# plainerman/DiffDock-Pocket

Hardware: AMD Instinct MI355X
Metric: ligand poses/sec (40 samples x 20 steps) on 3dpf (higher is better)
Workload: dtype f32 (fc and G products: fp16 hi/lo split of both operands on v_mfma_f32_16x16x32_f16 - the row-stationary conv kernel - and v_mfma_f32_32x32x16_f16, fp32 accumulate; G between its two kernels as fp16 hi + continuation byte = 19 significant bits; the exact fp32 MFMA form is timed in other_workloads)

## Files before the change

diffdock_pocket_amd/csrc/ddp_gemm.hip:

```cpp
#include <hip/hip_runtime.h>
#include <stdint.h>
#include <type_traits>
#include <stdlib.h>

#include "ddp_hip.h"
#include "ddp_internal.h"

typedef float f32x2 __attribute__((ext_vector_type(2)));
typedef float f32x4 __attribute__((ext_vector_type(4)));

#define DDP_GEMM_THREADS 256
#define DDP_GEMM_ROWS 128

struct GemmOffs {
  int off[DDP_MAX_GEMM_BATCH];
};

template <int KT, int CPL>
__global__ __launch_bounds__(DDP_GEMM_THREADS, 2) void ddp_stage_a_kernel(const float* __restrict__ x, int ldx, int nrows,
                                                                           const int32_t* __restrict__ rows,
                                                                           const int32_t* __restrict__ nrows_dev, int out_rows,
                                                                           const GemmOffs offs, const float* __restrict__ w,
                                                                           int k, int ncols, float* __restrict__ out, int ldo) {
  constexpr int KP = (KT > 0) ? KT / 2 : 32;
// ... 225 lines not shown

template <int KT>
__global__ __launch_bounds__(DDP_GEMM_THREADS, 2) void ddp_stage_a_x3_kernel(const float* __restrict__ x, int ldx, int nrows,
                                                                              const int32_t* __restrict__ rows,
                                                                              const int32_t* __restrict__ nrows_dev, int out_rows,
                                                                              int mrows, const GemmOffs offs,
                                                                              const __bf16* __restrict__ w3, int ncols,
                                                                              float* __restrict__ out, int ldo) {
  if (nrows_dev) nrows = min(nrows, *nrows_dev);
  if ((int)blockIdx.y * mrows >= nrows) return;
  constexpr int KP = (KT + 15) / 16 * 16, NS = KP / 16, CT = DDP_SA3_CT;
  constexpr int XS = KP + 8;
  constexpr int NV = (32 * KT / 4 + DDP_GEMM_THREADS - 1) / DDP_GEMM_THREADS;
  constexpr int TS = 36;
  constexpr int NM = NS * 6;
  __shared__ __attribute__((aligned(16))) __bf16 xt[2][3][32 * XS];
  __shared__ __attribute__((aligned(16))) float st[4][2][32 * TS];
  const int z = (int)blockIdx.z, tid = (int)threadIdx.x;
  const int wave = tid >> 6, lane = tid & 63, r = lane & 31, hh = lane >> 5;
  const int col0 = ((int)blockIdx.x * 4 + wave) * (32 * CT);
  bf16x8 wr[CT][3][NS];
#pragma unroll
  for (int t = 0; t < CT; ++t) {
    const int c = min(col0 + 32 * t + r, ncols - 1);
#pragma unroll
    for (int p = 0; p < 3; ++p)
#pragma unroll
      for (int s2 = 0; s2 < NS; ++s2)
        wr[t][p][s2] = *reinterpret_cast<const bf16x8*>(w3 + (((((size_t)z * 3 + p) * NS + s2) * 2 + hh) * ncols + c) * 8);
  }
  if constexpr (KP > KT) {
    for (int i = tid; i < 2 * 3 * 32 * (KP - KT); i += DDP_GEMM_THREADS) {
      const int kk = i % (KP - KT), rr = (i / (KP - KT)) % 32, bp = i / ((KP - KT) * 32);
      xt[bp / 3][bp % 3][rr * XS + KT + kk] = (__bf16)0.f;
    }
  }
  const float* __restrict__ xb = x + offs.off[z];
  for (int R0 = (int)blockIdx.y * mrows; R0 < nrows; R0 += (int)gridDim.y * mrows) {
  const int R1 = min(nrows, R0 + mrows);
  const bool al4 = ((ldx | offs.off[z]) & 3) == 0 && (reinterpret_cast<size_t>(x) & 15) == 0;
  f32x4 xv[NV];
  auto fetch = [&](int row0) {
#pragma unroll
    for (int v = 0; v < NV; ++v) {
      const int i = tid + v * DDP_GEMM_THREADS;
      const int rr = min(i / (KT / 4), 31), q = i % (KT / 4);
      const int ri = min(row0 + rr, nrows - 1);
      const float* __restrict__ p = xb + (size_t)(rows ? rows[ri] : ri) * ldx + 4 * q;
      if (al4)
        xv[v] = *reinterpret_cast<const f32x4*>(p);
      else
        xv[v] = f32x4{p[0], p[1], p[2], p[3]};
    }
  };
  auto park = [&](int buf) {
#pragma unroll
    for (int v = 0; v < NV; ++v) {
      const int i = tid + v * DDP_GEMM_THREADS;
      if (i < 32 * (KT / 4)) {
        const int rr = i / (KT / 4), q = i % (KT / 4);
        bf16x4 h, m, l;
#pragma unroll
        for (int e = 0; e < 4; ++e) {
          const float f = xv[v][e];
          h[e] = (__bf16)f;
          const float r1 = f - (float)h[e];
          m[e] = (__bf16)r1;
          l[e] = (__bf16)(r1 - (float)m[e]);
        }
        *reinterpret_cast<bf16x4*>(&xt[buf][0][rr * XS + 4 * q]) = h;
        *reinterpret_cast<bf16x4*>(&xt[buf][1][rr * XS + 4 * q]) = m;
        *reinterpret_cast<bf16x4*>(&xt[buf][2][rr * XS + 4 * q]) = l;
      }
    }
  };
  float* pend_ob = nullptr;
  int pend_c0 = 0, pend_rows = 0, pend_buf = 0, pbuf = 0;
  int pend_ri[4] = {0, 0, 0, 0};
  f32x4 dv = {0.f, 0.f, 0.f, 0.f};
  auto drain_read = [&](int p) {
    if (pend_ob) dv = *reinterpret_cast<const f32x4*>(&st[wave][pend_buf][(8 * p + (lane >> 3)) * TS + 4 * (lane & 7)]);
  };
  auto drain_store = [&](int p) {
    if (pend_ob) {
      const int rr = 8 * p + (lane >> 3), c = pend_c0 + 4 * (lane & 7);
      if (rr < pend_rows && c < ncols) *reinterpret_cast<f32x4*>(&pend_ob[(size_t)pend_ri[p] * ldo + c]) = dv;
    }
  };
  fetch(R0);
  park(0);
  __syncthreads();
  int buf = 0;
  for (int row0 = R0; row0 < R1; row0 += 32, buf ^= 1) {
    const bool more = row0 + 32 < R1;
    if (more) fetch(row0 + 32);
    bf16x8 a[3][NS];
#pragma unroll
    for (int p = 0; p < 3; ++p)
#pragma unroll
      for (int s2 = 0; s2 < NS; ++s2) a[p][s2] = *reinterpret_cast<const bf16x8*>(&xt[buf][p][r * XS + 16 * s2 + 8 * hh]);
    float* __restrict__ ob = out + (size_t)z * out_rows * ldo;
    int blk_ri[4];
#pragma unroll
    for (int p = 0; p < 4; ++p) {
      const int ri = min(row0 + 8 * p + (lane >> 3), R1 - 1);
      blk_ri[p] = rows ? rows[ri] : ri;
    }
#pragma unroll
    for (int t = 0; t < CT; ++t) {
      f32x16 acc;
#pragma unroll
      for (int i = 0; i < 16; ++i) acc[i] = 0.f;
#pragma unroll
      for (int m = 0; m < NM; ++m) {
        constexpr int PA[6] = {2, 0, 1, 1, 0, 0}, PB[6] = {0, 2, 1, 0, 1, 0};
        const int pr = m / NS, s2 = m % NS;
        acc = __builtin_amdgcn_mfma_f32_32x32x16_bf16(a[PA[pr]][s2], wr[t][PB[pr]][s2], acc, 0, 0, 0);
        static_assert(NM / 4 >= 3 && NM % 4 == 0, "quarter schedule");
        if (m % (NM / 4) == 0) drain_read(m / (NM / 4));
        if (m % (NM / 4) == 2) drain_store(m / (NM / 4));
      }
      float* tl = st[wave][pbuf];
#pragma unroll
      for (int i = 0; i < 16; ++i) tl[((i & 3) + 8 * (i >> 2) + 4 * hh) * TS + r] = acc[i];
      pend_ob = ob;
#pragma unroll
      for (int p = 0; p < 4; ++p) pend_ri[p] = blk_ri[p];
      pend_c0 = col0 + 32 * t;
      pend_rows = R1 - row0;
      pend_buf = pbuf;
      pbuf ^= 1;
    }
    if (more) park(buf ^ 1);
    __syncthreads();
  }
#pragma unroll
  for (int p = 0; p < 4; ++p) {
    drain_read(p);
    drain_store(p);
  }
  __syncthreads();
  }
}

typedef _Float16 h8 __attribute__((ext_vector_type(8)));
typedef _Float16 h4 __attribute__((ext_vector_type(4)));
#ifndef DDP_SAH_CT_GH
#define DDP_SAH_CT_GH 4
#endif
#ifndef DDP_SAH_CT
#define DDP_SAH_CT 4
#endif

template <int KT, bool GH = false, bool G3 = false>
__global__ __launch_bounds__(DDP_GEMM_THREADS, 2) void ddp_stage_a_h2_kernel(const float* __restrict__ x, int ldx, int nrows,
                                                                              const int32_t* __restrict__ rows,
                                                                              const int32_t* __restrict__ nrows_dev, int out_rows,
                                                                              int mrows, const GemmOffs offs,
                                                                              const _Float16* __restrict__ wh, int ncols,
                                                                              float* __restrict__ out, int ldo, int32_t* range_flag,
                                                                              const int32_t* __restrict__ gh_dest = nullptr) {
  if (nrows_dev) nrows = min(nrows, *nrows_dev);
  if ((int)blockIdx.y * mrows >= nrows) return;
  constexpr int KP = (KT + 15) / 16 * 16, NS = KP / 16, CT = GH ? DDP_SAH_CT_GH : DDP_SAH_CT;
  constexpr int XS = KP + 8;
  constexpr int NV = (32 * KT / 4 + DDP_GEMM_THREADS - 1) / DDP_GEMM_THREADS;
  constexpr int TS = 36;
  constexpr int RS3 = 392;
  __shared__ __attribute__((aligned(16))) _Float16 xt[2][2][32 * XS];
  __shared__ __attribute__((aligned(16))) float st[G3 ? 1 : 4][2][G3 ? 4 : 32 * TS];
  __shared__ __attribute__((aligned(16))) char g3t[G3 ? 4 : 1][G3 ? 32 * RS3 : 16];
  const int z = (int)blockIdx.z, tid = (int)threadIdx.x;
  const int wave = tid >> 6, lane = tid & 63, r = lane & 31, hh = lane >> 5;
  const int col0 = ((int)blockIdx.x * 4 + wave) * (32 * CT);
  h8 wr[CT][2][NS];
#pragma unroll
  for (int t = 0; t < CT; ++t) {
    const int c = min(col0 + 32 * t + r, ncols - 1);
#pragma unroll
    for (int p = 0; p < 2; ++p)
#pragma unroll
      for (int s2 = 0; s2 < NS; ++s2)
        wr[t][p][s2] = *reinterpret_cast<const h8*>(wh + (((((size_t)z * 2 + p) * NS + s2) * 2 + hh) * ncols + c) * 8);
  }
  if constexpr (KP > KT) {
    for (int i = tid; i < 2 * 2 * 32 * (KP - KT); i += DDP_GEMM_THREADS) {
      const int kk = i % (KP - KT), rr = (i / (KP - KT)) % 32, bp = i / ((KP - KT) * 32);
      xt[bp / 2][bp % 2][rr * XS + KT + kk] = (_Float16)0.f;
    }
  }
  const float* __restrict__ xb = x + offs.off[z];
  float* __restrict__ ob = out + (size_t)z * out_rows * ldo;
  int cq[CT];
#pragma unroll
  for (int t = 0; t < CT; ++t) cq[t] = max(0, min(4 * (lane & 7), ncols - 4 - (col0 + 32 * t)));
  int gh_o[CT][2];
  bool gh_sp[CT];
  float gh_max = 0.f;
#pragma unroll
  for (int t = 0; t < CT; ++t) {
    gh_o[t][0] = gh_o[t][1] = 0;
    gh_sp[t] = false;
    if constexpr (GH) {
      const int g = min(col0 + 32 * t + 8 * (lane & 3), ncols - 8) >> 3;
      const int32_t* __restrict__ d = gh_dest + ((size_t)z * (ncols >> 3) + g) * 2;
      gh_o[t][0] = d[0] & ~3;
      gh_o[t][1] = d[1];
      gh_sp[t] = (d[0] & 1) != 0;
    }
  }
  unsigned sp3 = 0u;
  int g3_rr[3] = {0, 0, 0}, g3_pc[3] = {0, 0, 0};
  if constexpr (G3) {
    const int g = min(col0 + 8 * (lane & 15), ncols - 8) >> 3;
    sp3 = (unsigned)__ballot((gh_dest[((size_t)z * (ncols >> 3) + g) * 2] & 1) != 0) & 0xffffu;
#pragma unroll
    for (int j = 0; j < 3; ++j) {
      g3_rr[j] = (64 * j + lane) / 24;
      g3_pc[j] = (64 * j + lane) % 24;
    }
  }
  for (int R0 = (int)blockIdx.y * mrows; R0 < nrows; R0 += (int)gridDim.y * mrows) {
  const int R1 = min(nrows, R0 + mrows);
  const bool al4 = ((ldx | offs.off[z]) & 3) == 0 && (reinterpret_cast<size_t>(x) & 15) == 0;
  f32x4 xv[NV];
  auto fetch = [&](int row0) {
#pragma unroll
    for (int v = 0; v < NV; ++v) {
      const int i = tid + v * DDP_GEMM_THREADS;
      const int rr = min(i / (KT / 4), 31), q = i % (KT / 4);
      const int ri = min(row0 + rr, nrows - 1);
      const float* __restrict__ p = xb + (size_t)(rows ? rows[ri] : ri) * ldx + 4 * q;
      if (al4)
        xv[v] = *reinterpret_cast<const f32x4*>(p);
      else
        xv[v] = f32x4{p[0], p[1], p[2], p[3]};
    }
  };
  auto park = [&](int buf) {
#pragma unroll
    for (int v = 0; v < NV; ++v) {
      const int i = tid + v * DDP_GEMM_THREADS;
      if (i < 32 * (KT / 4)) {
        const int rr = i / (KT / 4), q = i % (KT / 4);
        h4 h, l;
#pragma unroll
        for (int e = 0; e < 4; ++e) {
          const float f = GH ? xv[v][e] * (float)DDP_GH_SX : xv[v][e];
          if (!(fabsf(f) <= 65504.f) && range_flag) *range_flag = 1;
          h[e] = (_Float16)f;
          l[e] = (_Float16)(GH ? f - (float)h[e] : (f - (float)h[e]) * 2048.f);
        }
        *reinterpret_cast<h4*>(&xt[buf][0][rr * XS + 4 * q]) = h;
        *reinterpret_cast<h4*>(&xt[buf][1][rr * XS + 4 * q]) = l;
      }
    }
  };
  size_t pend_off[4] = {0, 0, 0, 0};
  int pend_lds[4] = {0, 0, 0, 0};
  bool pend_sp = false;
  int pbuf = 0;
  f32x4 dv = {0.f, 0.f, 0.f, 0.f};
  f32x4 dv2 = {0.f, 0.f, 0.f, 0.f};
  auto gh_read = [&](const float* pt, int p) {
    if (p & 1) {
      dv = dv2;
      return;
    }
    typedef float f32x8 __attribute__((ext_vector_type(8)));
    const f32x4 a = *reinterpret_cast<const f32x4*>(&pt[pend_lds[p]]), b = *reinterpret_cast<const f32x4*>(&pt[pend_lds[p] + 4]);
    const f32x8 f = {a[0], a[1], a[2], a[3], b[0], b[1], b[2], b[3]};
    const h8 hi = __builtin_convertvector(f, h8);
    const f32x8 rest = f - __builtin_convertvector(hi, f32x8);
    const h8 lo = __builtin_convertvector(rest, h8);
    const float m8 = fmaxf(fmaxf(fmaxf(fabsf(f[0]), fabsf(f[1])), fmaxf(fabsf(f[2]), fabsf(f[3]))), fmaxf(fmaxf(fabsf(f[4]), fabsf(f[5])), fmaxf(fabsf(f[6]), fabsf(f[7]))));
    gh_max = fmaxf(gh_max, pend_sp ? m8 : 0.f);
    const f32x4 vh = __builtin_bit_cast(f32x4, hi), vl = __builtin_bit_cast(f32x4, lo);
#pragma unroll
    for (int e = 0; e < 4; ++e) {
      dv[e] = pend_sp ? vh[e] : a[e];
      dv2[e] = pend_sp ? vl[e] : b[e];
    }
  };
  auto block = [&](auto drain_tag, int t, const h8 (&a)[2][NS], const int (&blk_ri)[4], int nr) {
    constexpr bool DRAIN = decltype(drain_tag)::value;
    f32x16 am, ac;
#pragma unroll
    for (int i = 0; i < 16; ++i) { am[i] = 0.f; ac[i] = 0.f; }
    const float* pt = st[wave][pbuf ^ 1];
#pragma unroll
    for (int s2 = 0; s2 < NS; ++s2) {
      if constexpr (DRAIN && NS == 4) {
        if constexpr (GH)
          gh_read(pt, s2);
        else
          dv = *reinterpret_cast<const f32x4*>(&pt[pend_lds[s2]]);
      }
      if constexpr (GH) {
        am = __builtin_amdgcn_mfma_f32_32x32x16_f16(wr[t][0][s2], a[0][s2], am, 0, 0, 0);
        am = __builtin_amdgcn_mfma_f32_32x32x16_f16(wr[t][1][s2], a[0][s2], am, 0, 0, 0);
        am = __builtin_amdgcn_mfma_f32_32x32x16_f16(wr[t][0][s2], a[1][s2], am, 0, 0, 0);
      } else {
        am = __builtin_amdgcn_mfma_f32_32x32x16_f16(a[0][s2], wr[t][0][s2], am, 0, 0, 0);
        ac = __builtin_amdgcn_mfma_f32_32x32x16_f16(a[0][s2], wr[t][1][s2], ac, 0, 0, 0);
        ac = __builtin_amdgcn_mfma_f32_32x32x16_f16(a[1][s2], wr[t][0][s2], ac, 0, 0, 0);
      }
      if constexpr (DRAIN && NS == 4) {
        {
          *reinterpret_cast<f32x4*>(&ob[pend_off[s2]]) = dv;
        }
      }
    }
    if constexpr (DRAIN && NS != 4) {
#pragma unroll
      for (int p = 0; p < 4; ++p) {
        if constexpr (GH)
          gh_read(pt, p);
        else
          dv = *reinterpret_cast<const f32x4*>(&pt[pend_lds[p]]);
        *reinterpret_cast<f32x4*>(&ob[pend_off[p]]) = dv;
      }
    }
    float* tl = st[wave][pbuf];
    if constexpr (GH) {
#pragma unroll
      for (int q4 = 0; q4 < 4; ++q4)
        *reinterpret_cast<f32x4*>(&tl[r * TS + 8 * q4 + 4 * hh]) = f32x4{am[4 * q4], am[4 * q4 + 1], am[4 * q4 + 2], am[4 * q4 + 3]};
    } else {
#pragma unroll
      for (int i = 0; i < 16; ++i) tl[((i & 3) + 8 * (i >> 2) + 4 * hh) * TS + r] = am[i] + ac[i] * (1.f / 2048.f);
    }
    if constexpr (GH) {
#if defined(DDP_GH_ABL) && DDP_GH_ABL == 1
      pend_sp = false;
#else
      pend_sp = gh_sp[t];
#endif
#pragma unroll
      for (int p = 0; p < 4; ++p) {
        const int rr = min(16 * (p >> 1) + (lane >> 2), nr - 1);
        pend_lds[p] = rr * TS + 8 * (lane & 3);
        pend_off[p] = (size_t)blk_ri[p >> 1] * ldo + gh_o[t][p & 1];
      }
    } else {
#pragma unroll
      for (int p = 0; p < 4; ++p) {
        const int rr = min(8 * p + (lane >> 3), nr - 1);
        pend_lds[p] = rr * TS + cq[t];
        pend_off[p] = (size_t)blk_ri[p] * ldo + (col0 + 32 * t + cq[t]);
      }
    }
    pbuf ^= 1;
  };
  auto block3 = [&](int t, const h8 (&a)[2][NS]) {
    f32x16 am;
#pragma unroll
    for (int i = 0; i < 16; ++i) am[i] = 0.f;
#pragma unroll
    for (int s2 = 0; s2 < NS; ++s2) {
      am = __builtin_amdgcn_mfma_f32_32x32x16_f16(wr[t][0][s2], a[0][s2], am, 0, 0, 0);
      am = __builtin_amdgcn_mfma_f32_32x32x16_f16(wr[t][1][s2], a[0][s2], am, 0, 0, 0);
      am = __builtin_amdgcn_mfma_f32_32x32x16_f16(wr[t][0][s2], a[1][s2], am, 0, 0, 0);
    }
    char* tl = g3t[G3 ? wave : 0] + r * RS3 + 96 * t;
#pragma unroll
    for (int q = 0; q < 4; ++q) {
      const bool sp = ((sp3 >> (4 * t + q)) & 1u) != 0u;
      const float v0 = am[4 * q], v1 = am[4 * q + 1], v2 = am[4 * q + 2], v3 = am[4 * q + 3];
      gh_max = fmaxf(gh_max, sp ? fmaxf(fmaxf(fabsf(v0), fabsf(v1)), fmaxf(fabsf(v2), fabsf(v3))) : 0.f);
      const uint32_t b0 = __builtin_bit_cast(uint32_t, v0) + 0x10u, b1 = __builtin_bit_cast(uint32_t, v1) + 0x10u;
      const uint32_t b2 = __builtin_bit_cast(uint32_t, v2) + 0x10u, b3 = __builtin_bit_cast(uint32_t, v3) + 0x10u;
      typedef __fp16 pk2 __attribute__((ext_vector_type(2)));
      const pk2 h01 = __builtin_amdgcn_cvt_pkrtz(__builtin_bit_cast(float, b0), __builtin_bit_cast(float, b1));
      const pk2 h23 = __builtin_amdgcn_cvt_pkrtz(__builtin_bit_cast(float, b2), __builtin_bit_cast(float, b3));
      const uint32_t lo = ((b0 >> 5) & 0xffu) | (((b1 >> 5) & 0xffu) << 8) | (((b2 >> 5) & 0xffu) << 16) | ((b3 >> 5) << 24);
      typedef uint32_t u32x2 __attribute__((ext_vector_type(2)));
      u32x2 w8;
      w8[0] = sp ? __builtin_bit_cast(uint32_t, h01) : __builtin_bit_cast(uint32_t, v0);
      w8[1] = sp ? __builtin_bit_cast(uint32_t, h23) : __builtin_bit_cast(uint32_t, v1);
      *reinterpret_cast<u32x2*>(tl + 24 * q + 8 * hh) = w8;
      *reinterpret_cast<uint32_t*>(tl + 24 * q + 16 + 4 * hh) = sp ? lo : __builtin_bit_cast(uint32_t, v2);
    }
  };
  auto drain3 = [&](int myrow, int nr) {
    __builtin_amdgcn_fence(__ATOMIC_RELEASE, "wavefront");
    __builtin_amdgcn_wave_barrier();
    const char* img = g3t[G3 ? wave : 0];
    float* __restrict__ oc = ob + 6 * (col0 >> 3);
#pragma unroll
    for (int p = 0; p < 4; ++p)
#pragma unroll
      for (int j = 0; j < 3; ++j) {
        const int rl = min(8 * p + g3_rr[j], nr - 1);
        typedef uint32_t u32x2 __attribute__((ext_vector_type(2)));
        const u32x2 lo8 = *reinterpret_cast<const u32x2*>(img + rl * RS3 + 16 * g3_pc[j]);
        const u32x2 hi8 = *reinterpret_cast<const u32x2*>(img + rl * RS3 + 16 * g3_pc[j] + 8);
        const int ri = __shfl(myrow, rl);
        typedef uint32_t u32x4 __attribute__((ext_vector_type(4)));
        *reinterpret_cast<u32x4*>(oc + (size_t)ri * ldo + 4 * g3_pc[j]) = u32x4{lo8[0], lo8[1], hi8[0], hi8[1]};
      }
    __builtin_amdgcn_wave_barrier();
  };
  fetch(R0);
  park(0);
  __syncthreads();
  int buf = 0;
  bool first = true;
  for (int row0 = R0; row0 < R1; row0 += 32, buf ^= 1) {
    const bool more = row0 + 32 < R1;
    if (more) fetch(row0 + 32);
    h8 a[2][NS];
#pragma unroll
    for (int p = 0; p < 2; ++p)
#pragma unroll
      for (int s2 = 0; s2 < NS; ++s2) a[p][s2] = *reinterpret_cast<const h8*>(&xt[buf][p][r * XS + 16 * s2 + 8 * hh]);
    int blk_ri[4];
#pragma unroll
    for (int p = 0; p < 4; ++p) {
      const int ri = min(row0 + (GH ? 16 * (p & 1) + (lane >> 2) : 8 * p + (lane >> 3)), R1 - 1);
      blk_ri[p] = rows ? rows[ri] : ri;
    }
    const int nr = R1 - row0;
    if constexpr (G3) {
      if (col0 < ncols) {
        const int ri = min(row0 + r, R1 - 1);
        const int myrow = rows ? rows[ri] : ri;
#pragma unroll
        for (int t = 0; t < CT; ++t) block3(t, a);
        drain3(myrow, nr);
      }
      if (more) park(buf ^ 1);
      __syncthreads();
      continue;
    }
#pragma unroll
    for (int t = 0; t < CT; ++t) {
      if (col0 + 32 * t >= ncols) continue;
      if (t == 0 && first)
        block(std::false_type{}, t, a, blk_ri, nr);
      else
        block(std::true_type{}, t, a, blk_ri, nr);
      first = false;
    }
    if (more) park(buf ^ 1);
    __syncthreads();
  }
  if (!first) {
    const float* pt = st[wave][pbuf ^ 1];
#pragma unroll
    for (int p = 0; p < 4; ++p) {
      if constexpr (GH)
        gh_read(pt, p);
      else
        dv = *reinterpret_cast<const f32x4*>(&pt[pend_lds[p]]);
      *reinterpret_cast<f32x4*>(&ob[pend_off[p]]) = dv;
    }
  }
  __syncthreads();
  }
  if constexpr (GH) {
    if (!(gh_max <= 65504.f) && range_flag) *range_flag = 1;
  }
}

static int stage_a_impl(const float* x, int ldx, int nrows, const int32_t* rows, const int32_t* nrows_dev, int out_rows,
                        const int32_t* offs, int nbatch, const float* w, const void* w_bf16x3, const void* w_h2, int k, int ncols, float* out,
                        int ldo, int32_t* range_flag, void* stream, const int32_t* gh_dest = nullptr, int gh_fmt = 0) {
  if (!rows) out_rows = nrows;
  if (out_rows < 1 && nrows > 0) return ddp_fail(DDP_EINVAL, "ddp_stage_a: out_rows");
  if (nbatch < 0 || nbatch > DDP_MAX_GEMM_BATCH) return ddp_fail(DDP_ELIMIT, "ddp_stage_a: nbatch > DDP_MAX_GEMM_BATCH");
  if (k < 2 || k > 64 || (k & 1)) return ddp_fail(DDP_ELIMIT, "ddp_stage_a: K must be even and in [2, 64]");
  if (ncols < 1 || nrows < 0 || (ldo < ncols && !(gh_dest && gh_fmt == 1 && ldo >= (ncols / 8) * 6)))
    return ddp_fail(DDP_EINVAL, "ddp_stage_a: ncols / nrows / ldo");
  if (gh_dest && gh_fmt == 1 && ((ncols & 127) != 0 || (ldo & 31) != 0))
    return ddp_fail(DDP_EINVAL, "ddp_stage_a_gh3: ncols % 128 == 0 (a wave's four column blocks), ldo % 32 == 0 (whole 128-byte lines)");
  if (nbatch == 0 || nrows == 0) return 0;
  if (!x || !offs || !w || !out) return ddp_fail(DDP_EINVAL, "ddp_stage_a: null argument");
  if ((reinterpret_cast<size_t>(x) & 3) || (reinterpret_cast<size_t>(out) & 7))
    return ddp_fail(DDP_EINVAL, "ddp_stage_a: x must be 4-byte aligned, out 8-byte aligned");
  GemmOffs O;
  for (int i = 0; i < DDP_MAX_GEMM_BATCH; ++i) O.off[i] = (i < nbatch) ? offs[i] : 0;
  hipStream_t s = (hipStream_t)stream;
  const int nry = (nrows + DDP_GEMM_ROWS - 1) / DDP_GEMM_ROWS;
#define DDP_GEMM_LAUNCH(KT, CPL)                                                                                 \
  hipLaunchKernelGGL((ddp_stage_a_kernel<KT, CPL>), dim3((ncols + CPL * DDP_GEMM_THREADS - 1) / (CPL * DDP_GEMM_THREADS), nry, nbatch), \
                     dim3(DDP_GEMM_THREADS), 0, s, x, ldx, nrows, rows, nrows_dev, out_rows, O, w, k, ncols, out, ldo)
  const bool wide = ((ncols | ldo) & 3) == 0 && ncols >= 4 * DDP_GEMM_THREADS && (reinterpret_cast<size_t>(out) & 15) == 0;
#define DDP_GEMM_MFMA(KT)                                                                                        \
  hipLaunchKernelGGL((ddp_stage_a_mfma_kernel<KT>), dim3((ncols + 128 * DDP_SA_CT - 1) / (128 * DDP_SA_CT), gy, nbatch), \
                     dim3(DDP_GEMM_THREADS), 0, s, x, ldx, nrows, rows, nrows_dev, out_rows, mrows, O, w, ncols, out, ldo)
  const bool listed = rows && nrows_dev;
  int mrows = listed ? (nrows >= 16384 ? 256 : 128) : (nrows >= 8192 ? DDP_GEMM_MROWS : nrows >= 384 ? 256 : 64);
  int gy = (nrows + mrows - 1) / mrows;
  if (listed && gy > 96) gy = 96;
#ifdef DDP_SA_TUNE
  if (nrows < 8192 || listed) {
    if (const char* e = getenv("DDP_SA_MROWS")) mrows = atoi(e);
    gy = (nrows + mrows - 1) / mrows;
    const char* c = getenv("DDP_SA_GYCAP");
    const int cap = c ? atoi(c) : 96;
    if (listed && gy > cap) gy = cap;
  }
#endif
  static const bool no_mfma = getenv("DDP_STAGE_A_VALU") != nullptr;
  if (gh_dest) {
    if (!(w_h2 && wide && (k == 60 || k == 32 || k == 24 || k == 16) && (reinterpret_cast<size_t>(w_h2) & 15) == 0 && (ncols & 31) == 0 &&
          (reinterpret_cast<size_t>(gh_dest) & 7) == 0))
      return ddp_fail(DDP_EINVAL, "ddp_stage_a_gh: plane output needs the h2 path (w_h2, k in {60, 32, 24, 16}) and ncols % 32 == 0");
    const dim3 grid((ncols + 128 * DDP_SAH_CT_GH - 1) / (128 * DDP_SAH_CT_GH), gy, nbatch);
    const int pad = ddp_shape_stage_a_pad;
    static int pad_have[8] = {0, 0, 0, 0, 0, 0, 0, 0};
#define DDP_GEMM_GH(KT, I)                                                                                       \
    {                                                                                                            \
      if (pad > 0) {                                                                                             \
        const hipError_t ep = (gh_fmt == 1) ? ddp_need_lds(reinterpret_cast<const void*>(ddp_stage_a_h2_kernel<KT, true, true>), pad, &pad_have[4 + I]) \
                                            : ddp_need_lds(reinterpret_cast<const void*>(ddp_stage_a_h2_kernel<KT, true>), pad, &pad_have[I]); \
        if (ep != hipSuccess) return ddp_fail_hip(ep, "hipFuncSetAttribute(stage A)");                           \
      }                                                                                                          \
      if (gh_fmt == 1)                                                                                           \
        hipLaunchKernelGGL((ddp_stage_a_h2_kernel<KT, true, true>), grid, dim3(DDP_GEMM_THREADS), pad, s, x, ldx, nrows, rows, nrows_dev, out_rows, mrows, O, \
                           reinterpret_cast<const _Float16*>(w_h2), ncols, out, ldo, range_flag, gh_dest);       \
      else                                                                                                       \
        hipLaunchKernelGGL((ddp_stage_a_h2_kernel<KT, true>), grid, dim3(DDP_GEMM_THREADS), pad, s, x, ldx, nrows, rows, nrows_dev, out_rows, mrows, O, \
                           reinterpret_cast<const _Float16*>(w_h2), ncols, out, ldo, range_flag, gh_dest);       \
    }
    switch (k) {
      case 60: DDP_GEMM_GH(60, 0); break;
      case 32: DDP_GEMM_GH(32, 1); break;
      case 24: DDP_GEMM_GH(24, 2); break;
      default: DDP_GEMM_GH(16, 3); break;
    }
#undef DDP_GEMM_GH
    const hipError_t eg = hipGetLastError();
    if (eg != hipSuccess) return ddp_fail_hip(eg, "ddp_stage_a_gh launch");
    return 0;
  }
  if (w_h2 && wide && (k == 60 || k == 32 || k == 24 || k == 16) && !no_mfma && (reinterpret_cast<size_t>(w_h2) & 15) == 0) {
    const dim3 grid((ncols + 128 * DDP_SAH_CT - 1) / (128 * DDP_SAH_CT), gy, nbatch);
#define DDP_GEMM_H2(KT)                                                                                          \
    hipLaunchKernelGGL((ddp_stage_a_h2_kernel<KT>), grid, dim3(DDP_GEMM_THREADS), 0, s, x, ldx, nrows, rows, nrows_dev, out_rows, mrows, O, \
                       reinterpret_cast<const _Float16*>(w_h2), ncols, out, ldo, range_flag)
    switch (k) {
      case 60: DDP_GEMM_H2(60); break;
      case 32: DDP_GEMM_H2(32); break;
      case 24: DDP_GEMM_H2(24); break;
      default: DDP_GEMM_H2(16); break;
    }
#undef DDP_GEMM_H2
    const hipError_t eh = hipGetLastError();
    if (eh != hipSuccess) return ddp_fail_hip(eh, "ddp_stage_a (h2) launch");
    return 0;
  }
  if (w_bf16x3 && wide && (k == 60 || k == 32) && !no_mfma && (reinterpret_cast<size_t>(w_bf16x3) & 15) == 0) {
    const dim3 grid((ncols + 128 * DDP_SA3_CT - 1) / (128 * DDP_SA3_CT), gy, nbatch);
    if (k == 60)
      hipLaunchKernelGGL((ddp_stage_a_x3_kernel<60>), grid, dim3(DDP_GEMM_THREADS), 0, s, x, ldx, nrows, rows, nrows_dev, out_rows, mrows, O,
                         reinterpret_cast<const __bf16*>(w_bf16x3), ncols, out, ldo);
    else
      hipLaunchKernelGGL((ddp_stage_a_x3_kernel<32>), grid, dim3(DDP_GEMM_THREADS), 0, s, x, ldx, nrows, rows, nrows_dev, out_rows, mrows, O,
                         reinterpret_cast<const __bf16*>(w_bf16x3), ncols, out, ldo);
    const hipError_t e3 = hipGetLastError();
    if (e3 != hipSuccess) return ddp_fail_hip(e3, "ddp_stage_a (bf16x3) launch");
    return 0;
  }
  if (ncols >= 512 && !no_mfma && (k == 60 || k == 64 || k == 32 || k == 24 || k == 16)) {
    switch (k) {
      case 60: DDP_GEMM_MFMA(60); break;
      case 64: DDP_GEMM_MFMA(64); break;
      case 32: DDP_GEMM_MFMA(32); break;
      case 24: DDP_GEMM_MFMA(24); break;
      default: DDP_GEMM_MFMA(16); break;
    }
  } else
  switch (k) {
    case 60: if (wide) DDP_GEMM_LAUNCH(60, 4); else DDP_GEMM_LAUNCH(60, 2); break;
    case 32: DDP_GEMM_LAUNCH(32, 2); break;
    case 24: DDP_GEMM_LAUNCH(24, 2); break;
    case 16: DDP_GEMM_LAUNCH(16, 2); break;
    default: DDP_GEMM_LAUNCH(0, 2); break;
  }
#undef DDP_GEMM_LAUNCH
#undef DDP_GEMM_MFMA
  const hipError_t err = hipGetLastError();
  if (err != hipSuccess) return ddp_fail_hip(err, "ddp_stage_a launch");
  return 0;
}

extern "C" int ddp_stage_a(const float* x, int ldx, int nrows, const int32_t* rows, const int32_t* nrows_dev, int out_rows,
                           const int32_t* offs, int nbatch, const float* w, const void* w_bf16x3, int k, int ncols, float* out, int ldo,
                           void* stream) {
  return stage_a_impl(x, ldx, nrows, rows, nrows_dev, out_rows, offs, nbatch, w, w_bf16x3, nullptr, k, ncols, out, ldo, nullptr, stream);
}

extern "C" int ddp_stage_a_h2(const float* x, int ldx, int nrows, const int32_t* rows, const int32_t* nrows_dev, int out_rows,
                              const int32_t* offs, int nbatch, const float* w, const void* w_h2, int k, int ncols, float* out, int ldo,
                              int32_t* range_flag, void* stream) {
  return stage_a_impl(x, ldx, nrows, rows, nrows_dev, out_rows, offs, nbatch, w, nullptr, w_h2, k, ncols, out, ldo, range_flag, stream);
}

extern "C" int ddp_stage_a_gh(const float* x, int ldx, int nrows, const int32_t* rows, const int32_t* nrows_dev, int out_rows,
                              const int32_t* offs, int nbatch, const float* w, const void* w_h2, int k, int ncols, float* out, int ldo,
                              int32_t* range_flag, const int32_t* dest, void* stream) {
  if (!dest) return ddp_fail(DDP_EINVAL, "ddp_stage_a_gh: dest");
  return stage_a_impl(x, ldx, nrows, rows, nrows_dev, out_rows, offs, nbatch, w, nullptr, w_h2, k, ncols, out, ldo, range_flag, stream, dest);
}

extern "C" int ddp_stage_a_gh3(const float* x, int ldx, int nrows, const int32_t* rows, const int32_t* nrows_dev, int out_rows,
                               const int32_t* offs, int nbatch, const float* w, const void* w_h2, int k, int ncols, float* out, int ldo,
                               int32_t* range_flag, const int32_t* dest, void* stream) {
  if (!dest) return ddp_fail(DDP_EINVAL, "ddp_stage_a_gh3: dest");
  return stage_a_impl(x, ldx, nrows, rows, nrows_dev, out_rows, offs, nbatch, w, nullptr, w_h2, k, ncols, out, ldo, range_flag, stream, dest, 1);
}
```

include/ddp_hip.h:

```cpp
#ifndef DDP_HIP_H
#define DDP_HIP_H

#include <stdint.h>

#ifdef __cplusplus
extern "C" {
#endif

#define DDP_ABI_VERSION 17
#define DDP_EINVAL (-1)
#define DDP_ELIMIT (-2)

#define DDP_MAX_TASKS 9
#define DDP_MAX_BLOCKS 4
#define DDP_MAX_SEGS 3
#define DDP_MAX_NS 64
#define DDP_EDGE_TILE 64

enum ddp_feat_kind {
  DDP_F_SCALAR_S0 = 0,
  DDP_F_DOT = 1,
  DDP_F_SCALAR_S1 = 2,
  DDP_F_VEC_S0 = 3,
  DDP_F_CROSS = 4
// ... 61 lines not shown
  float* msg;
  const float* g[2];
  const int32_t* pos;
  const int32_t* n_edges_dev;
  const void* w1h;
  const void* w2h;
  int32_t* h2_range_flag;
  const void* wsh;
  const float* bsp;
  const void* gh[2];
  int32_t gh_fmt;
  int32_t rows_form;
  int32_t rows_bias_k;
  int32_t rows_seg0, rows_seg1, rows_nts;
} ddp_conv_task_t;
#define DDP_ROWS_SX 16
#define DDP_ROWS_SW 256
#define DDP_ROWS_SH 16
#define DDP_ROWS_SG 32
#define DDP_ROWS_KPERM(ks, hh, i) (32 * ((ks) >> 1) + ((8 * ((ks) & 1) + (i)) & 3) + 8 * ((8 * ((ks) & 1) + (i)) >> 2) + 4 * (hh))
#define DDP_ROWS16_POS(j) (16 * (((j) & 7) >> 2) + 4 * ((j) >> 3) + ((j) & 3))
#define DDP_GH3_LD(hid, gcp) ((((((hid) + 7) / 8) * (gcp) + ((gcp) + 5) / 6 + 15) / 16) * 96)
#define DDP_GH_LD(hid, gcp) ((((((hid) + 7) / 8) * 8 + 1) * (gcp) + 31) / 32 * 32)
int ddp_conv_messages(const ddp_conv_shape_t* shape, const ddp_conv_task_t* tasks, int ntasks, void* stream);

int ddp_conv_rows(const ddp_conv_shape_t* shape, const ddp_conv_task_t* tasks, int ntasks, void* stream);

typedef struct {
  const float* msg;
  const int32_t* rowptr;
  const float* bn_scale;
  const float* bn_shift;
  int32_t n_edges;
  const int32_t* rowmap;
  const int32_t* n_edges_dev;
} ddp_reduce_src_t;
int ddp_segment_reduce(float* x, int ldx, int n_nodes, int d_out, const ddp_reduce_src_t* srcs, int nsrc,
                       int accumulate, int n_rep, int rep_stride, void* stream);

int ddp_edge_featurize(const float* pos_a, const int32_t* ia, const float* pos_b, const int32_t* ib, int n_edges,
                       const int32_t* n_edges_dev, const float* offset, int k_rbf, float coeff, const float* pre,
                       const int32_t* pre_idx, int ld_pre, const float* pre2, int n_pre2, int ld_pre2, const float* w1d,
                       const float* w2, const float* b2, int ns, float* out, float* sh, void* stream);

#define DDP_MAX_FEATURIZE_JOBS 8
typedef struct {
  const float* pos_a;
  const int32_t* ia;
  const float* pos_b;
  const int32_t* ib;
  int32_t n_edges;
  const int32_t* n_edges_dev;
  const float* offset;
  int32_t k_rbf;
  float coeff;
  const float* pre;
  const int32_t* pre_idx;
  int32_t ld_pre;
  const float* pre2;
  int32_t n_pre2, ld_pre2;
  const float* w1d;
  const float* w2;
  const float* b2;
  int32_t ns;
  float* out;
  float* sh;
} ddp_featurize_job_t;
int ddp_edge_featurize_jobs(const ddp_featurize_job_t* jobs, int njobs, void* stream);

int ddp_torsion_sh(const float* sh_edge, const float* bond_vec, const int32_t* bond_of_edge, int n_edges,
                   const int32_t* n_edges_dev, float* out, const float* x, int ldx, int ns, const int32_t* b0,
                   const int32_t* b1, int n_bonds, float* bond_attr, void* stream);

typedef struct {
  const float* t[4];
  int32_t t_stride[4];
  float sig_min[4], sig_max[4];
  float* sigma[4];
  int32_t n_graphs;
  float* cut;
  float cut_mul, cut_add;
  float* graph_emb;
  int32_t sd;
  float emb_scale;
  const float* freq;
  const float* lig_pos;
  const int32_t* graph_ptr;
  float* center;
  struct {
    const float* pos;
    const int32_t* b0;
    const int32_t* b1;
    int32_t n;
    float* mid;
    float* vec;
  } bonds[2];
  struct {
    const int32_t* src;
    int32_t* dst;
    int32_t n;
  } copy[2];
} ddp_prologue_args_t;
int ddp_step_prologue(const ddp_prologue_args_t* args, void* stream);

typedef struct {
  const float* gp;
  int32_t ld_gp, n_graphs, ns, sd;
  const float* graph_emb;
  const float* w1[2];
  const float* b1[2];
  const float* w2[2];
  const float* b2[2];
  const float* sigma[2];
  const float* so3_table;
  int32_t so3_n;
  float so3_lo, so3_span;
  float* out[2];
} ddp_trrot_args_t;
int ddp_trrot_head(const ddp_trrot_args_t* args, void* stream);

typedef struct {
  const float* h;
  int32_t ld_h, n_bonds, ns;
  const float* w1;
  const float* w2;
  const float* sigma;
  const int32_t* graph_of_bond;
  const float* torus_table;
  int32_t torus_n;
  float torus_lo, torus_span;
  float* out;
} ddp_tor_args_t;
int ddp_tor_head(const ddp_tor_args_t* args, void* stream);

#define DDP_MAX_GEMM_BATCH 16
#define DDP_G_LD(hid, gcols) ((((((hid) + 3) / 4) * 4 + 1) * (gcols) + 31) / 32 * 32)
int ddp_stage_a(const float* x, int ldx, int nrows, const int32_t* rows, const int32_t* nrows_dev, int out_rows, const int32_t* offs,
                int nbatch, const float* w, const void* w_bf16x3, int k, int ncols, float* out, int ldo, void* stream);

int ddp_stage_a_h2(const float* x, int ldx, int nrows, const int32_t* rows, const int32_t* nrows_dev, int out_rows, const int32_t* offs,
                   int nbatch, const float* w, const void* w_h2, int k, int ncols, float* out, int ldo, int32_t* range_flag, void* stream);
int ddp_stage_a_gh(const float* x, int ldx, int nrows, const int32_t* rows, const int32_t* nrows_dev, int out_rows, const int32_t* offs,
                   int nbatch, const float* w, const void* w_h2, int k, int ncols, float* out, int ldo, int32_t* range_flag,
                   const int32_t* dest, void* stream);

int ddp_stage_a_gh3(const float* x, int ldx, int nrows, const int32_t* rows, const int32_t* nrows_dev, int out_rows, const int32_t* offs,
                    int nbatch, const float* w, const void* w_h2, int k, int ncols, float* out, int ldo, int32_t* range_flag,
                    const int32_t* dest, void* stream);

#define DDP_GH_SX 2

int ddp_set_occupancy_shaping(int rows_min_lds_bytes, int stage_a_lds_pad_bytes);

int ddp_pose_update(const float* pos_in, int n_samples, int n_atoms, const float* tr, const float* rot, const float* tor,
                    int n_tor, const int32_t* bonds, const uint8_t* mask_rotate, float* pos_out, void* stream);

int ddp_sidechain_update(const float* pos_in, int n_samples, int n_atoms, const float* angles, int n_bonds,
                         const int32_t* edge_idx, const int32_t* subcomponents, const int32_t* mapping, float* pos_out,
                         void* stream);

typedef struct {
  const float* score[4];
  const float* z[4];
  float* out[4];
  int32_t n[4];
} ddp_sde_args_t;
int ddp_sde_update(const float* coef, const ddp_sde_args_t* args, void* stream);

#define DDP_RADIUS_DROP_SELF 1
#define DDP_RADIUS_NEAREST 2
int ddp_radius_count(const float* x, const int32_t* x_ptr, const float* y, const int32_t* y_batch, int ny, float r,
                     int max_neighbors, int flags, int32_t* counts, void* stream);
int ddp_radius_fill(const float* x, const int32_t* x_ptr, const float* y, const int32_t* y_batch, int ny, float r,
                    int max_neighbors, int flags, const int32_t* offsets, int32_t* out_query, int32_t* out_x, void* stream);
int ddp_knn(const float* x, const int32_t* x_ptr, const int32_t* batch, int n, int k, int32_t* out_neighbors, void* stream);

int ddp_group_by_key(const int32_t* key, int n_items, int n_keys, const int32_t* pay0, const int32_t* pay1, const int32_t* pay2,
                     int32_t* rowptr, int32_t* perm, int32_t* out_key, int32_t* out0, int32_t* out1, int32_t* out2,
                     int32_t* scratch, void* stream);

#define DDP_MAX_LIST_JOBS 12

typedef struct {
  int32_t n;
  const int32_t* n_dev;
  const int32_t* flag;
  const int32_t* val;
  const int32_t* rowptr;
  int32_t base;
  int32_t* excl;
  int32_t* excl2;
  int32_t* list;
  int32_t* total;
} ddp_scan_job_t;
int ddp_scan_jobs(const ddp_scan_job_t* jobs, int njobs, void* stream);

typedef struct {
  const int32_t* idx;
  int32_t n;
  const int32_t* n_dev;
  int32_t* mask;
} ddp_mark_job_t;
int ddp_mark_jobs(const ddp_mark_job_t* jobs, int njobs, void* stream);

typedef struct {
  int32_t n_rows;
  const int32_t* keep;
  const int32_t* old_rowptr;
  const int32_t* new_rowptr;
  const int32_t* in[3];
  int32_t* out[3];
} ddp_rowcopy_job_t;
int ddp_rowcopy_jobs(const ddp_rowcopy_job_t* jobs, int njobs, void* stream);

typedef struct {
  int32_t n;
  const int32_t* n_dev;
  const int32_t* mask_a;
  const int32_t* idx_a;
  const int32_t* mask_b;
  const int32_t* idx_b;
  int32_t* out_idx;
  const int32_t* pay[4];
  int32_t pay_add[4];
  int32_t* out[4];
  int32_t* total;
  int32_t* block_count;
  int32_t* block_off;
} ddp_select_job_t;
int ddp_select_jobs(const ddp_select_job_t* jobs, int njobs, void* stream);

int ddp_gather_rows(const float* x, int ldx, const int32_t* idx, int n, const int32_t* n_dev, float* out, int ldo, int ncols,
                    void* stream);

int ddp_clean_pair_maps(const int32_t* touched, const int32_t* recv, const int32_t* src, const int32_t* rowptr, int n_edges, int e0,
                        int n_graphs, int n0, int32_t* rowmap, int32_t* rows_v, void* stream);

int ddp_flex_mark(const float* pos, const int32_t* flag, int n_b_per_graph, const int32_t* a, const int32_t* b, int n_edges, int e0,
                  int n_a_per_graph, int a_too, int ref_list, int32_t* mark, void* stream);
int ddp_fallback_rowmap(const int32_t* mark, const int32_t* recv, const int32_t* old_rowptr, const int32_t* new_rowptr, int n_edges,
                        int n_recv_per_graph, int32_t* rowmap, void* stream);

typedef struct {
  const float* x;
  const int32_t* x_ptr;
  const float* y;
  const int32_t* y_batch;
  int32_t ny;
  float r;
  int32_t max_neighbors;
  int32_t flags;
  const float* graph_div;
  int32_t* counts;
  int32_t* offsets;
  int32_t base;
  int32_t* total;
  int32_t* out_query;
  int32_t* out_x;
  int32_t capacity;
  int32_t* overflow;
} ddp_radius_job_t;
int ddp_radius_search_jobs(const ddp_radius_job_t* jobs, int njobs, void* stream);

typedef struct {
  const int32_t* key;
  int32_t n_items;
  const int32_t* n_items_dev;
  int32_t n_keys;
  const int32_t* pay[3];
  int32_t* rowptr;
  int32_t* perm;
  int32_t* out_key;
  int32_t* out[3];
  const int32_t* key_map;
  int32_t* scratch;
} ddp_group_job_t;
int ddp_group_by_key_jobs(const ddp_group_job_t* jobs, int njobs, void* stream);

#define DDP_MAX_NODE_JOBS 8
#define DDP_MAX_NODE_CAT 16
typedef struct {
  int32_t n_rows;
  const int32_t* cat;
  int32_t ld_cat, n_cat;
  const float* table;
  int32_t feat_off[DDP_MAX_NODE_CAT];
  int32_t emb_dim, emb_mode;
  const float* dense[2];
  int32_t ld_dense[2], n_dense[2];
  const float* t;
  int32_t t_stride;
  float scale;
  const float* freq;
  const float* sig_emb;
  int32_t ld_sig, sd;
  float* sig_out;
  int32_t ld_sig_out;
  const float* w;
  const float* bias;
  float* out;
  int32_t ld_out, ncols, zero_to;
  const float* add;
  int32_t ld_add;
} ddp_node_job_t;
int ddp_node_linear(const ddp_node_job_t* jobs, int njobs, void* stream);

// ... 229 lines not shown
```

Measured before the change: 175.0.

## Add warp-specialized stage A G3 kernel with dedicated store-drain wave

Adds a new stage-A GEMM kernel for the G3 plane-output format. Three waves run the fp16 hi/lo MFMA blocks over 384-column tiles with double-buffered x staging, and a fourth wave only drains the LDS images to global memory, so stores overlap with compute. The host also caps the grid's y dimension to a persistent-style count based on CU slots, and the MFMA block is factored into a shared helper. The new path is gated to large row counts and can be toggled with an env var. The trade-off is one wave no longer doing MFMA, plus extra barriers per tile.

After: 178.7 (median of 6 runs). 2.1% higher.

```diff
diff --git a/diffdock_pocket_amd/csrc/ddp_gemm.hip b/diffdock_pocket_amd/csrc/ddp_gemm.hip
--- a/diffdock_pocket_amd/csrc/ddp_gemm.hip
+++ b/diffdock_pocket_amd/csrc/ddp_gemm.hip
@@ -401,6 +401,37 @@
 #define DDP_SAH_CT 4
 #endif
 
+template <int NS>
+__device__ __forceinline__ void sa_g3_block(const h8 (&w)[2][NS], const h8 (&a)[2][NS], char* tl, unsigned sp4, int hh, float& gh_max) {
+  f32x16 am;
+#pragma unroll
+  for (int i = 0; i < 16; ++i) am[i] = 0.f;
+#pragma unroll
+  for (int s2 = 0; s2 < NS; ++s2) {
+    am = __builtin_amdgcn_mfma_f32_32x32x16_f16(w[0][s2], a[0][s2], am, 0, 0, 0);
+    am = __builtin_amdgcn_mfma_f32_32x32x16_f16(w[1][s2], a[0][s2], am, 0, 0, 0);
+    am = __builtin_amdgcn_mfma_f32_32x32x16_f16(w[0][s2], a[1][s2], am, 0, 0, 0);
+  }
+#pragma unroll
+  for (int q = 0; q < 4; ++q) {
+    const bool sp = ((sp4 >> q) & 1u) != 0u;
+    const float v0 = am[4 * q], v1 = am[4 * q + 1], v2 = am[4 * q + 2], v3 = am[4 * q + 3];
+    gh_max = fmaxf(gh_max, sp ? fmaxf(fmaxf(fabsf(v0), fabsf(v1)), fmaxf(fabsf(v2), fabsf(v3))) : 0.f);
+    const uint32_t b0 = __builtin_bit_cast(uint32_t, v0) + 0x10u, b1 = __builtin_bit_cast(uint32_t, v1) + 0x10u;
+    const uint32_t b2 = __builtin_bit_cast(uint32_t, v2) + 0x10u, b3 = __builtin_bit_cast(uint32_t, v3) + 0x10u;
+    typedef __fp16 pk2 __attribute__((ext_vector_type(2)));
+    const pk2 h01 = __builtin_amdgcn_cvt_pkrtz(__builtin_bit_cast(float, b0), __builtin_bit_cast(float, b1));
+    const pk2 h23 = __builtin_amdgcn_cvt_pkrtz(__builtin_bit_cast(float, b2), __builtin_bit_cast(float, b3));
+    const uint32_t lo = ((b0 >> 5) & 0xffu) | (((b1 >> 5) & 0xffu) << 8) | (((b2 >> 5) & 0xffu) << 16) | ((b3 >> 5) << 24);
+    typedef uint32_t u32x2 __attribute__((ext_vector_type(2)));
+    u32x2 w8;
+    w8[0] = sp ? __builtin_bit_cast(uint32_t, h01) : __builtin_bit_cast(uint32_t, v0);
+    w8[1] = sp ? __builtin_bit_cast(uint32_t, h23) : __builtin_bit_cast(uint32_t, v1);
+    *reinterpret_cast<u32x2*>(tl + 24 * q + 8 * hh) = w8;
+    *reinterpret_cast<uint32_t*>(tl + 24 * q + 16 + 4 * hh) = sp ? lo : __builtin_bit_cast(uint32_t, v2);
+  }
+}
+
 template <int KT, bool GH = false, bool G3 = false>
 __global__ __launch_bounds__(DDP_GEMM_THREADS, 2) void ddp_stage_a_h2_kernel(const float* __restrict__ x, int ldx, int nrows,
                                                                               const int32_t* __restrict__ rows,
@@ -602,34 +633,7 @@
     pbuf ^= 1;
   };
   auto block3 = [&](int t, const h8 (&a)[2][NS]) {
-    f32x16 am;
-#pragma unroll
-    for (int i = 0; i < 16; ++i) am[i] = 0.f;
-#pragma unroll
-    for (int s2 = 0; s2 < NS; ++s2) {
-      am = __builtin_amdgcn_mfma_f32_32x32x16_f16(wr[t][0][s2], a[0][s2], am, 0, 0, 0);
-      am = __builtin_amdgcn_mfma_f32_32x32x16_f16(wr[t][1][s2], a[0][s2], am, 0, 0, 0);
-      am = __builtin_amdgcn_mfma_f32_32x32x16_f16(wr[t][0][s2], a[1][s2], am, 0, 0, 0);
-    }
-    char* tl = g3t[G3 ? wave : 0] + r * RS3 + 96 * t;
-#pragma unroll
-    for (int q = 0; q < 4; ++q) {
-      const bool sp = ((sp3 >> (4 * t + q)) & 1u) != 0u;
-      const float v0 = am[4 * q], v1 = am[4 * q + 1], v2 = am[4 * q + 2], v3 = am[4 * q + 3];
-      gh_max = fmaxf(gh_max, sp ? fmaxf(fmaxf(fabsf(v0), fabsf(v1)), fmaxf(fabsf(v2), fabsf(v3))) : 0.f);
-      const uint32_t b0 = __builtin_bit_cast(uint32_t, v0) + 0x10u, b1 = __builtin_bit_cast(uint32_t, v1) + 0x10u;
-      const uint32_t b2 = __builtin_bit_cast(uint32_t, v2) + 0x10u, b3 = __builtin_bit_cast(uint32_t, v3) + 0x10u;
-      typedef __fp16 pk2 __attribute__((ext_vector_type(2)));
-      const pk2 h01 = __builtin_amdgcn_cvt_pkrtz(__builtin_bit_cast(float, b0), __builtin_bit_cast(float, b1));
-      const pk2 h23 = __builtin_amdgcn_cvt_pkrtz(__builtin_bit_cast(float, b2), __builtin_bit_cast(float, b3));
-      const uint32_t lo = ((b0 >> 5) & 0xffu) | (((b1 >> 5) & 0xffu) << 8) | (((b2 >> 5) & 0xffu) << 16) | ((b3 >> 5) << 24);
-      typedef uint32_t u32x2 __attribute__((ext_vector_type(2)));
-      u32x2 w8;
-      w8[0] = sp ? __builtin_bit_cast(uint32_t, h01) : __builtin_bit_cast(uint32_t, v0);
-      w8[1] = sp ? __builtin_bit_cast(uint32_t, h23) : __builtin_bit_cast(uint32_t, v1);
-      *reinterpret_cast<u32x2*>(tl + 24 * q + 8 * hh) = w8;
-      *reinterpret_cast<uint32_t*>(tl + 24 * q + 16 + 4 * hh) = sp ? lo : __builtin_bit_cast(uint32_t, v2);
-    }
+    sa_g3_block<NS>(wr[t], a, g3t[G3 ? wave : 0] + r * RS3 + 96 * t, (sp3 >> (4 * t)) & 0xfu, hh, gh_max);
   };
   auto drain3 = [&](int myrow, int nr) {
     __builtin_amdgcn_fence(__ATOMIC_RELEASE, "wavefront");
@@ -710,6 +714,219 @@
   if constexpr (GH) {
     if (!(gh_max <= 65504.f) && range_flag) *range_flag = 1;
   }
+}
+
+#define DDP_SA_BAR()                                   \
+  do {                                                 \
+    asm volatile("s_waitcnt lgkmcnt(0)" ::: "memory"); \
+    __builtin_amdgcn_s_barrier();                      \
+    asm volatile("" ::: "memory");                     \
+  } while (0)
+template <int KT>
+__global__ __launch_bounds__(DDP_GEMM_THREADS, 2) void ddp_stage_a_g3dw_kernel(const float* __restrict__ x, int ldx, int nrows,
+                                                                                const int32_t* __restrict__ rows,
+                                                                                const int32_t* __restrict__ nrows_dev, int out_rows,
+                                                                                int mrows, const GemmOffs offs,
+                                                                                const _Float16* __restrict__ wh, int ncols,
+                                                                                float* __restrict__ out, int ldo, int32_t* range_flag,
+                                                                                const int32_t* __restrict__ gh_dest) {
+  static_assert(DDP_GEMM_THREADS == 256, "3 MFMA waves + 1 store wave");
+  if (nrows_dev) nrows = min(nrows, *nrows_dev);
+  if ((int)blockIdx.y * mrows >= nrows) return;
+  constexpr int KP = (KT + 15) / 16 * 16, NS = KP / 16;
+  constexpr int XS = KP + 8, RS3 = 392;
+  constexpr int NP = 32 * (KT / 4);
+  constexpr int NMT = 192, NV = (NP + NMT - 1) / NMT;
+  __shared__ __attribute__((aligned(16))) _Float16 xt[2][2][32 * XS];
+  __shared__ __attribute__((aligned(16))) char img[3][32 * RS3];
+  __shared__ int32_t rowid[2][32];
+  const int z = (int)blockIdx.z, tid = (int)threadIdx.x;
+  const int wave = __builtin_amdgcn_readfirstlane(tid >> 6), lane = tid & 63, r = lane & 31, hh = lane >> 5;
+  const int colw = (int)blockIdx.x * 384;
+  const int ngr = min(3, (ncols - colw) >> 7);
+  if constexpr (KP > KT) {
+    for (int i = tid; i < 2 * 2 * 32 * (KP - KT); i += DDP_GEMM_THREADS) {
+      const int kk = i % (KP - KT), rr = (i / (KP - KT)) % 32, bp = i / ((KP - KT) * 32);
+      xt[bp / 2][bp % 2][rr * XS + KT + kk] = (_Float16)0.f;
+    }
+  }
+  struct Tile { int R0, R1, row0; };
+  const int ystep = (int)gridDim.y * mrows;
+  auto tile_next = [&](Tile t) {
+    t.row0 += 32;
+    if (t.row0 >= t.R1) {
+      t.R0 += ystep;
+      t.row0 = t.R0;
+      t.R1 = min(nrows, t.R0 + mrows);
+    }
+    return t;
+  };
+  const Tile tile0 = {(int)blockIdx.y * mrows, min(nrows, (int)blockIdx.y * mrows + mrows), (int)blockIdx.y * mrows};
+  if (wave == 3) {
+    float* __restrict__ ob = out + (size_t)z * out_rows * ldo + 6 * (colw >> 3);
+    int dl[12];
+    size_t doff[12];
+#pragma unroll
+    for (int k = 0; k < 12; ++k) { dl[k] = 0; doff[k] = 0; }
+    auto drain = [&](int g) {
+      const char* im = img[g];
+      float* __restrict__ og = ob + 96 * g;
+#pragma unroll
+      for (int k = 0; k < 12; ++k) {
+        typedef uint32_t u32x2 __attribute__((ext_vector_type(2)));
+        typedef uint32_t u32x4 __attribute__((ext_vector_type(4)));
+        const u32x2 lo8 = *reinterpret_cast<const u32x2*>(im + dl[k]);
+        const u32x2 hi8 = *reinterpret_cast<const u32x2*>(im + dl[k] + 8);
+        *reinterpret_cast<u32x4*>(og + doff[k]) = u32x4{lo8[0], lo8[1], hi8[0], hi8[1]};
+      }
+    };
+    Tile t = tile0;
+    DDP_SA_BAR();
+    for (int n = 0;; ++n) {
+      if (n > 0 && ngr > 2) drain(2);
+      DDP_SA_BAR();
+      {
+        const int nr = t.R1 - t.row0;
+#pragma unroll
+        for (int k = 0; k < 12; ++k) {
+          const int i = 64 * (k % 3) + lane, rl = min(8 * (k / 3) + i / 24, nr - 1);
+          dl[k] = rl * RS3 + 16 * (i % 24);
+          doff[k] = (size_t)rowid[n & 1][rl] * ldo + 4 * (i % 24);
+        }
+      }
+      DDP_SA_BAR();
+      drain(0);
+      DDP_SA_BAR();
+      if (ngr > 1) drain(1);
+      DDP_SA_BAR();
+      t = tile_next(t);
+      if (t.row0 >= nrows) break;
+    }
+    if (ngr > 2) drain(2);
+    return;
+  }
+  h8 wr[4][2][NS];
+#pragma unroll
+  for (int j = 0; j < 4; ++j) {
+    const int c = min(colw + 32 * (3 * j + wave) + r, ncols - 1);
+#pragma unroll
+    for (int p = 0; p < 2; ++p)
+#pragma unroll
+      for (int s2 = 0; s2 < NS; ++s2)
+        wr[j][p][s2] = *reinterpret_cast<const h8*>(wh + (((((size_t)z * 2 + p) * NS + s2) * 2 + hh) * ncols + c) * 8);
+  }
+  unsigned sp3;
+  {
+    const int l = lane & 15;
+    const int g = min(((colw + 32 * (3 * (l >> 2) + wave)) >> 3) + (l & 3), (ncols >> 3) - 1);
+    sp3 = (unsigned)__ballot((gh_dest[((size_t)z * (ncols >> 3) + g) * 2] & 1) != 0) & 0xffffu;
+  }
+  float gh_max = 0.f;
+  const float* __restrict__ xb = x + offs.off[z];
+  const bool al4 = ((ldx | offs.off[z]) & 3) == 0 && (reinterpret_cast<size_t>(x) & 15) == 0;
+  auto run = [&](auto listed_tag, auto al4_tag) {
+  constexpr bool LISTED = decltype(listed_tag)::value, AL4 = decltype(al4_tag)::value;
+  f32x4 xv[NV];
+  int xrow[NV], xnext[NV];
+  auto rows_of = [&](int row0, int (&dst)[NV]) {
+#pragma unroll
+    for (int v = 0; v < NV; ++v) {
+      const int i = min(tid + v * NMT, NP - 1);
+      const int ri = min(row0 + i / (KT / 4), nrows - 1);
+      if constexpr (LISTED)
+        dst[v] = rows[ri];
+      else
+        dst[v] = ri;
+    }
+  };
+  auto fetch = [&]() {
+#pragma unroll
+    for (int v = 0; v < NV; ++v) {
+      const int i = min(tid + v * NMT, NP - 1);
+      const float* __restrict__ p = xb + (size_t)xrow[v] * ldx + 4 * (i % (KT / 4));
+      if constexpr (AL4)
+        xv[v] = *reinterpret_cast<const f32x4*>(p);
+      else
+        xv[v] = f32x4{p[0], p[1], p[2], p[3]};
+    }
+  };
+  auto park = [&](int buf) {
+#pragma unroll
+    for (int v = 0; v < NV; ++v) {
+      const int i = tid + v * NMT;
+      if (i < NP) {
+        const int rr = i / (KT / 4), q = i % (KT / 4);
+        h4 h, l;
+#pragma unroll
+        for (int e = 0; e < 4; ++e) {
+          const float f = xv[v][e] * (float)DDP_GH_SX;
+          if (!(fabsf(f) <= 65504.f) && range_flag) *range_flag = 1;
+          h[e] = (_Float16)f;
+          l[e] = (_Float16)(f - (float)h[e]);
+        }
+        *reinterpret_cast<h4*>(&xt[buf][0][rr * XS + 4 * q]) = h;
+        *reinterpret_cast<h4*>(&xt[buf][1][rr * XS + 4 * q]) = l;
+        if (q == 0) rowid[buf][rr] = xrow[v];
+      }
+    }
+  };
+  {
+    Tile t1 = tile_next(tile0), t2 = tile_next(t1);
+    rows_of(tile0.row0, xrow);
+    fetch();
+    park(0);
+    rows_of(t1.row0, xnext);
+    DDP_SA_BAR();
+    for (int n = 0;; ++n) {
+      const int buf = n & 1;
+      const bool more = t1.row0 < nrows;
+      if (more) {
+#pragma unroll
+        for (int v = 0; v < NV; ++v) xrow[v] = xnext[v];
+        fetch();
+        rows_of(t2.row0, xnext);
+      }
+      h8 a[2][NS];
+#pragma unroll
+      for (int p = 0; p < 2; ++p)
+#pragma unroll
+        for (int s2 = 0; s2 < NS; ++s2) a[p][s2] = *reinterpret_cast<const h8*>(&xt[buf][p][r * XS + 16 * s2 + 8 * hh]);
+#pragma unroll
+      for (int j = 0; j < 4; ++j) {
+        const int b = 3 * j + wave;
+        if ((b >> 2) < ngr)
+          sa_g3_block<NS>(wr[j], a, img[b >> 2] + r * RS3 + 96 * (b & 3), (sp3 >> (4 * j)) & 0xfu, hh, gh_max);
+        if (j == 3 && more) park(buf ^ 1);
+        DDP_SA_BAR();
+      }
+      if (!more) break;
+      t1 = t2;
+      t2 = tile_next(t2);
+    }
+  }
+  };
+  if (rows) {
+    if (al4)
+      run(std::true_type{}, std::true_type{});
+    else
+      run(std::true_type{}, std::false_type{});
+  } else {
+    if (al4)
+      run(std::false_type{}, std::true_type{});
+    else
+      run(std::false_type{}, std::false_type{});
+  }
+  if (!(gh_max <= 65504.f) && range_flag) *range_flag = 1;
+}
+
+extern "C" int ddp_sa_drainwave;
+int ddp_sa_drainwave = -1;
+static int stage_a_drainwave() {
+  if (ddp_sa_drainwave < 0) {
+    const char* e = getenv("DDP_SA_DRAINWAVE");
+    ddp_sa_drainwave = (e && e[0] == '0') ? 0 : (e && e[0] == '2') ? 2 : 1;
+  }
+  return ddp_sa_drainwave;
 }
 
 static int stage_a_impl(const float* x, int ldx, int nrows, const int32_t* rows, const int32_t* nrows_dev, int out_rows,
@@ -753,14 +970,44 @@
 #endif
   static const bool no_mfma = getenv("DDP_STAGE_A_VALU") != nullptr;
   if (gh_dest) {
-    if (!(w_h2 && wide && (k == 60 || k == 32 || k == 24 || k == 16) && (reinterpret_cast<size_t>(w_h2) & 15) == 0 && (ncols & 31) == 0 &&
+    const bool wide_gh = gh_fmt == 1 ? (((ncols | ldo) & 3) == 0 && (reinterpret_cast<size_t>(out) & 15) == 0) : wide;
+    if (!(w_h2 && wide_gh && (k == 60 || k == 32 || k == 24 || k == 16) && (reinterpret_cast<size_t>(w_h2) & 15) == 0 && (ncols & 31) == 0 &&
           (reinterpret_cast<size_t>(gh_dest) & 7) == 0))
       return ddp_fail(DDP_EINVAL, "ddp_stage_a_gh: plane output needs the h2 path (w_h2, k in {60, 32, 24, 16}) and ncols % 32 == 0");
-    const dim3 grid((ncols + 128 * DDP_SAH_CT_GH - 1) / (128 * DDP_SAH_CT_GH), gy, nbatch);
+    const int dw_mode = gh_fmt == 1 ? stage_a_drainwave() : 0;
+    const bool dw = dw_mode == 2 || (dw_mode == 1 && nrows >= (listed ? 16384 : 4096));
+    if (dw && !listed) {
+      static int slots = 0;
+      if (!slots) {
+        int dev = 0, ncu = 0;
+        if (hipGetDevice(&dev) != hipSuccess || hipDeviceGetAttribute(&ncu, hipDeviceAttributeMultiprocessorCount, dev) != hipSuccess || ncu < 1)
+          return ddp_fail(DDP_EINVAL, "ddp_stage_a_gh3: hipDeviceGetAttribute(multiprocessor count)");
+        slots = 2 * ncu;
+      }
+      mrows = 128;
+      gy = (nrows + mrows - 1) / mrows;
+      const int per_y = (int)((ncols + 383) / 384) * nbatch;
+      int best = 0;
+      double best_fill = 0.;
+      for (int kk = 1; kk <= 6 && best_fill < 0.95; ++kk) {
+        const int g = kk * slots / per_y;
+        const double fill = (double)g * per_y / ((double)kk * slots);
+        if (g >= 1 && fill > best_fill) { best = g; best_fill = fill; }
+      }
+      if (best >= 1 && gy > best) gy = best;
+    }
+    const dim3 grid(dw ? (ncols + 383) / 384 : (ncols + 128 * DDP_SAH_CT_GH - 1) / (128 * DDP_SAH_CT_GH), gy, nbatch);
     const int pad = ddp_shape_stage_a_pad;
-    static int pad_have[8] = {0, 0, 0, 0, 0, 0, 0, 0};
+    static int pad_have[12] = {0, 0, 0, 0, 0, 0, 0, 0, 0, 0, 0, 0};
 #define DDP_GEMM_GH(KT, I)                                                                                       \
-    {                                                                                                            \
+    if (dw) {                                                                                                    \
+      if (pad > 0) {                                                                                             \
+        const hipError_t ep = ddp_need_lds(reinterpret_cast<const void*>(ddp_stage_a_g3dw_kernel<KT>), pad, &pad_have[8 + I]); \
+        if (ep != hipSuccess) return ddp_fail_hip(ep, "hipFuncSetAttribute(stage A)");                           \
+      }                                                                                                          \
+      hipLaunchKernelGGL((ddp_stage_a_g3dw_kernel<KT>), grid, dim3(DDP_GEMM_THREADS), pad, s, x, ldx, nrows, rows, nrows_dev, out_rows, mrows, O, \
+                         reinterpret_cast<const _Float16*>(w_h2), ncols, out, ldo, range_flag, gh_dest);         \
+    } else {                                                                                                     \
       if (pad > 0) {                                                                                             \
         const hipError_t ep = (gh_fmt == 1) ? ddp_need_lds(reinterpret_cast<const void*>(ddp_stage_a_h2_kernel<KT, true, true>), pad, &pad_have[4 + I]) \
                                             : ddp_need_lds(reinterpret_cast<const void*>(ddp_stage_a_h2_kernel<KT, true>), pad, &pad_have[I]); \
diff --git a/include/ddp_hip.h b/include/ddp_hip.h
--- a/include/ddp_hip.h
+++ b/include/ddp_hip.h
@@ -237,6 +237,8 @@
 
 int ddp_set_occupancy_shaping(int rows_min_lds_bytes, int stage_a_lds_pad_bytes);
 
+extern int ddp_sa_drainwave;
+
 int ddp_pose_update(const float* pos_in, int n_samples, int n_atoms, const float* tr, const float* rot, const float* tor,
                     int n_tor, const int32_t* bonds, const uint8_t* mask_rotate, float* pos_out, void* stream);
 
```
